# anand-12/botorch

Measured on AMD Instinct MI355X. Metric: acq-evals/sec (q x restarts x MC), qEI forward, higher is better.
Workload: dtype f64; 1 GPU; C3 qEI forward: SingleTaskGP n=4096 d=6, q=16, 512 restarts/GPU, 512 Sobol MC samples, best_f = max(Y) - 1.5; n=4096, d=6, q=16, restarts_per_gpu=512, mc=512, parallelism=restart-sharded x1

## Files before the change

botorch_amd/csrc/post.hip:

```cpp
#include "common.h"
#include "post_wide_sched.h"

#include <algorithm>
#include <atomic>
#include <cstdlib>
#include <map>
#include <mutex>
#include <tuple>
#include <vector>

namespace {

constexpr int PC = 128;
constexpr int PI = 128;
constexpr int PK = 16;
constexpr int PLD = 144;
constexpr int DP = 8;
constexpr int kSlots = 512;
constexpr int kTileDoubles = 32 * 64;
#ifndef KXT_K
#define KXT_K 16
#endif

template <int KIND, int ND>
__device__ __forceinline__ double eval_kernel_row(const double (&xi)[ND], const double* __restrict__ Xt,
                                                  int n, int k, double outputscale, bool ivalid) {
  if (k >= n || !ivalid) return 0.0;
  const double* xt = Xt + (int64_t)k * DP;
  double d2 = 0.0;
#pragma unroll
  for (int t = 0; t < ND; ++t) {
    const double df = xi[t] - xt[t];
    d2 = fma(df, df, d2);
  }
#ifdef BO_PROBE_CHEAP_KERNEL
  return outputscale * d2 * 0.0;
#else
  return outputscale * kernel_from_d2<KIND>(d2);
#endif
}

__host__ __device__ __forceinline__ int splitk_chunks(int ci, int n, int kc_len) {
  const int e = ci * PC + PC;
  const int kfull = n < e ? n : e;
  return (kfull + kc_len - 1) / kc_len;
}
__host__ __device__ __forceinline__ int64_t splitk_base(int ci, int n, int kc_len) {
  int64_t s = 0;
  for (int c = 0; c < ci; ++c) s += splitk_chunks(c, n, kc_len);
  return s;
}

__device__ __forceinline__ void post_store_rt(const v4d (&acc)[8], int ci, int row0, int lane,
                                              int nI, double* __restrict__ Rt) {
  const int c0 = ci * PC;
  const int nrows_pad = nI * PI;
#pragma unroll
  for (int ct = 0; ct < 8; ++ct)
#pragma unroll
    for (int r = 0; r < 4; ++r) {
      const int c = c0 + ct * 16 + mfma_row(lane, r);
      Rt[(int64_t)c * nrows_pad + row0 + mfma_col(lane)] = acc[ct][r];
    }
}

__device__ __forceinline__ void post_epilogue(const v4d (&acc)[8], int ci, int row0, int lane,
                                              int n, const double* __restrict__ beta, int nI,
                                              double* __restrict__ Spart,
                                              double* __restrict__ mpart) {
  const int c0 = ci * PC;
  const int nrows16 = nI * (PI / 16);
  const int nrows_pad = nI * PI;
  v4d P = v4d_zero();
#pragma unroll
  for (int ct = 0; ct < 8; ++ct)
#pragma unroll
    for (int r = 0; r < 4; ++r) P = mfma_f64(acc[ct][r], acc[ct][r], P);
  double* sp = Spart + ((int64_t)ci * nrows16 + row0 / 16) * 256;
#pragma unroll
  for (int r = 0; r < 4; ++r) sp[mfma_row(lane, r) * 16 + mfma_col(lane)] = P[r];

  double m = 0.0;
#pragma unroll
  for (int ct = 0; ct < 8; ++ct)
#pragma unroll
    for (int r = 0; r < 4; ++r) {
      const int c = c0 + ct * 16 + mfma_row(lane, r);
      m = fma(acc[ct][r], (c < n) ? beta[c] : 0.0, m);
    }
  m += __shfl_xor(m, 16);
  m += __shfl_xor(m, 32);
  if (lane < 16) mpart[(int64_t)ci * nrows_pad + row0 + lane] = m;
}

struct FusedDx {
  const double* dmean;
  const double* dcov;
  const double* alpha;
  const double* Xq;
  const double* Xt;
  double ystd, outputscale;
  int B, q, Qp;
  double* part;
};

constexpr int POST_MAXM = 8;
struct PostMembers {
  const double* U[POST_MAXM];
  const double* beta[POST_MAXM];
  const double* Kt[POST_MAXM];
  double* Spart[POST_MAXM];
  double* mpart[POST_MAXM];
  double* Rt[POST_MAXM];
  int nm;
};

#ifndef BO_POST_PAIRED_REV
#define BO_POST_PAIRED_REV 1
#endif
#ifndef BO_USTORE_ALWAYS
#define BO_USTORE_ALWAYS 1
#endif
#ifndef BO_POST_RING
#define BO_POST_RING 1
#endif
template <int KIND, int ND, bool SPLIT, bool CROSS, bool PRE = false, bool LOWERK = false,
          bool FUSEDX = false>
__global__ __launch_bounds__(256, 2) void post_partials_kernel(
    const double* __restrict__ Xq, int nrows, const double* __restrict__ Xt, int n,
    const double* __restrict__ U, int64_t ldu, const double* __restrict__ beta,
    double outputscale, int nC, int nI, double* __restrict__ Spart, double* __restrict__ mpart,
    double* __restrict__ Rt, const int4* __restrict__ segs, const int* __restrict__ wg_off,
    double* __restrict__ work, const double* __restrict__ Qc, int rq, int64_t ldq,
    double* __restrict__ Cx, const double* __restrict__ Kt, int grouped, FusedDx fx = FusedDx{},
    int rt_blk = 0, PostMembers pm = PostMembers{}) {
  constexpr bool RING = PRE && BO_POST_RING;
  __shared__ __attribute__((aligned(16))) double Us[RING ? 3 : 2][PK][PLD];
  __shared__ __attribute__((aligned(16))) double Ks[2][PK][PLD];

  const int bid = blockIdx.x;
  int ci = 0, ii = 0, kbeg = 0, kend = 0;
  int ci_long = 0, ci_short = 0;
  if constexpr (SPLIT) {
  } else if (grouped == 2) {
    const int xcd = bid & 7;
    const int slot = bid >> 3;
    const int t = (slot >> 6) * 8 + xcd;
    const int w = slot & 63;
    const int nIG = nI >> 3;
    const int p = t / nIG;
    if (p >= (nC >> 4)) return;
    ci_long = ((nC >> 3) - 1 - p) * 8 + 7 - (w & 7);
    ci_short = p * 8 + (w & 7);
    ii = (t % nIG) * 8 + (w >> 3);
  } else if (grouped) {
    const int xcd = bid & 7;
    const int slot = bid >> 3;
    const int t = (slot >> 6) * 8 + xcd;
    const int w = slot & 63;
    const int nIG = nI >> 3;
    const int cg = (nC >> 3) - 1 - t / nIG;
    if (cg < 0) return;
    ci = cg * 8 + 7 - (w & 7);
    ii = (t % nIG) * 8 + (w >> 3);
    kend = min(n, ci * PC + PC);
  } else {
    const int xcd = bid & 7;
    const int slot = bid >> 3;
    const int jj = slot / nI;
    ii = slot - jj * nI;
    const int pos = jj * 8 + xcd;
    if (pos >= nC) return;
    ci = nC - 1 - pos;
    kend = min(n, ci * PC + PC);
  }
  if (LOWERK && !SPLIT && grouped != 2) {
    ci = nC - 1 - ci;
    kbeg = ci * PC;
    kend = n;
  }
  const double* const U_all = U;
  const double* const beta_all = beta;
  const double* const Kt_all = Kt;
  double* const Spart_all = Spart;
  double* const mpart_all = mpart;
  double* const Rt_all = Rt;
  int sbeg = 0, send = 1;
  if constexpr (SPLIT) {
    sbeg = wg_off[bid];
    send = wg_off[bid + 1];
  } else {
    if (grouped == 2) send = 2;
// ... 454 lines not shown
  }}
#define BO_W_STORE(G)                                                              \
  {_Pragma("unroll") for (int e = 0; e < SS; ++e) {                               \
    double* dst = &Us[(G) & (postw::kStages - 1)][e * PK + wave][2 * lane];        \
    *reinterpret_cast<double2*>(dst) = make_double2(us_[e][0], us_[e][1]);         \
    *reinterpret_cast<double2*>(dst + 8 * PLD) = make_double2(us_[e][2], us_[e][3]); \
  }}
#define BO_W_LOAD_B(UNIT, DST)                                                     \
  {                                                                                \
    const int u_ = min(max((UNIT), 0), 2 * nsteps - 1);                            \
    const double* bp = bbase + (int64_t)postw::unit_step(u_) * bstep +             \
                       (int64_t)(postw::unit_slice0(u_) * 4) * ldk;                \
    _Pragma("unroll") for (int it = 0; it < 2; ++it)                              \
      _Pragma("unroll") for (int sl = 0; sl < 2; ++sl)                               \
        DST[it][sl] = bp[(int64_t)(4 * sl) * ldk + it * 16];                         \
  }
#define BO_W_UADDR(UNIT)                                                           \
  (&Us[postw::stage_of_step(postw::unit_step(UNIT))]                               \
      [postw::stage_row_of_step(postw::unit_step(UNIT), PK) +                      \
       postw::unit_slice0(UNIT) * 4 + (lane >> 4)][lane & 15])
#define BO_W_PREF(UNIT)                                                            \
  {                                                                                \
    const double* us = BO_W_UADDR(UNIT);                                           \
    _Pragma("unroll") for (int ct = 0; ct < 8; ++ct) an[ct] = us[ct * 16];        \
  }
#define BO_W_UNIT(UNIT, BOP, PREF, DIAG)                                           \
  {                                                                                \
    const double* us = BO_W_UADDR(UNIT);                                           \
    const int kd = kfirst + postw::unit_step(UNIT) * kdir - c0;                    \
    const int ctb = (DIAG) ? __builtin_amdgcn_readfirstlane(max(kd, 0) >> 4) : 0;  \
    _Pragma("unroll") for (int sl = 0; sl < 2; ++sl) {                             \
      double a[8];                                                                 \
      _Pragma("unroll") for (int ct = 0; ct < 8; ++ct)                            \
        a[ct] = ((PREF) && sl == 0) ? an[ct] : us[sl * 4 * PLD + ct * 16];         \
      _Pragma("unroll") for (int ct = 0; ct < 8; ++ct)                            \
        if (!(DIAG) || ct >= ctb) {                                                \
          _Pragma("unroll") for (int it = 0; it < 2; ++it)                        \
            acc[ct][it] = mfma_f64(a[ct], BOP[it][sl], acc[ct][it]);              \
        }                                                                          \
    }                                                                              \
  }
#define BO_W_INTERVAL(J, DIAG, GUARD, STORE)                                       \
  {                                                                                \
    const int u0 = NU * (J) - lag;                                                 \
    if (!late) BO_W_PREF(u0);   \
    _Pragma("unroll") for (int k = 0; k < NU; ++k) {                              \
      if (!(GUARD) || postw::unit_valid(u0 + k, nsteps))                           \
        BO_W_UNIT(u0 + k, bu[k & 1], k == 0, DIAG)                                 \
      BO_W_LOAD_B(u0 + k + 2, bu[k & 1]);                                          \
      if ((STORE) && k == postw::store_after_unit(true) && late) BO_W_STORE((J) + 1);  \
    }                                                                              \
    if (late) BO_W_PREF(u0 + NU);               \
    if ((STORE) && !late) BO_W_STORE((J) + 1);                                     \
    if (STORE) BO_W_LOAD_U((J) + 2);             \
    __syncthreads();                                                               \
  }
    static_assert(postw::unit_at(3, 1, false) == 3 * NU + 1 &&
                      postw::unit_at(3, 1, true) == 3 * NU + 1 - postw::kLag &&
                      postw::store_after_unit(false) == NU - 1,
                  "BO_W_INTERVAL's units and stores are post_wide_sched.h's");

    BO_W_LOAD_U(0);
#pragma unroll
    for (int k = 0; k < 2; ++k) BO_W_LOAD_B(k - lag, bu[k]);
    BO_W_STORE(0);
    BO_W_LOAD_U(1);
    __syncthreads();
    const int jfull = nsteps / SS;
    constexpr int LB = postw::kLag > 1 ? (postw::kLag + 1) / 2 : 1;
    const int jd0 = min(jfull, max(1, d0 / SS));
    const int jd1 = max(jd0, min(jfull, (d1 + LB - 1) / SS + 1));
    int j = 0;
    BO_W_INTERVAL(j, 1, 1, 1)
    for (j = 1; j < jd0; ++j) BO_W_INTERVAL(j, 0, 0, 1)
    for (; j < jd1; ++j) BO_W_INTERVAL(j, 1, 0, 1)
    for (; j < jfull; ++j) BO_W_INTERVAL(j, 0, 0, 1)
    if (j < nss) {
      BO_W_INTERVAL(j, 1, 1, 1)
    }
    BO_W_INTERVAL(nss, 1, 1, 0)
#undef BO_W_INTERVAL
#undef BO_W_UNIT
#undef BO_W_PREF
#undef BO_W_UADDR
#undef BO_W_LOAD_B
#undef BO_W_STORE
#undef BO_W_LOAD_U

    const int nrows_pad = nI * PI;
    if (Rt != nullptr && rt_blk) {
#pragma unroll
      for (int ct = 0; ct < 8; ++ct)
#pragma unroll
        for (int it = 0; it < 2; ++it) {
          double* blk = Rt + ((int64_t)((c0 >> 4) + ct) * nrows16 +
                              ((i0 + wave * 32 + it * 16) >> 4)) * 256 + lane;
#pragma unroll
          for (int r = 0; r < 4; ++r) blk[r * 64] = acc[ct][it][r];
        }
    } else if (Rt != nullptr) {
#pragma unroll
      for (int ct = 0; ct < 8; ++ct)
#pragma unroll
        for (int it = 0; it < 2; ++it)
#pragma unroll
          for (int r = 0; r < 4; ++r) {
            const int c = c0 + ct * 16 + mfma_row(lane, r);
            const int i = i0 + wave * 32 + it * 16 + mfma_col(lane);
            Rt[(int64_t)c * nrows_pad + i] = acc[ct][it][r];
          }
    }
#pragma unroll
    for (int it = 0; it < 2; ++it) {
      v4d P = v4d_zero();
#pragma unroll
      for (int ct = 0; ct < 8; ++ct)
#pragma unroll
        for (int r = 0; r < 4; ++r) P = mfma_f64(acc[ct][it][r], acc[ct][it][r], P);
      const int row0 = i0 + wave * 32 + it * 16;
      double* sp = Spart + ((int64_t)ci * nrows16 + row0 / 16) * 256;
#pragma unroll
      for (int r = 0; r < 4; ++r) sp[mfma_row(lane, r) * 16 + mfma_col(lane)] = P[r];
      double m = 0.0;
#pragma unroll
      for (int ct = 0; ct < 8; ++ct)
#pragma unroll
        for (int r = 0; r < 4; ++r) {
          const int c = c0 + ct * 16 + mfma_row(lane, r);
          m = fma(acc[ct][it][r], (c < n) ? beta[c] : 0.0, m);
        }
      m += __shfl_xor(m, 16);
      m += __shfl_xor(m, 32);
      if (lane < 16) mpart[(int64_t)ci * nrows_pad + row0 + lane] = m;
    }
  }
}

struct RowsFromX {
  const double* X;
  const double* ls;
  int B, q, d, Qp;
  double* Xq_out;
};

struct KxtMembers {
  const double* ls[8];
  const double* Xt[8];
  double os[8];
  double* Xq[8];
  double* Kt[8];
  int nm;
};

template <int KIND, int ND, int KK = KXT_K, bool FROMX = false>
__global__ __launch_bounds__(256) void kxt_build_kernel(const double* __restrict__ Xq, int nrows,
                                                        const double* __restrict__ Xt, int n,
                                                        int np, int nrows_pad, double outputscale,
                                                        double* __restrict__ Kt,
                                                        RowsFromX rx = RowsFromX{},
                                                        KxtMembers km = KxtMembers{}) {
  if (km.nm > 0) {
    const int m = blockIdx.z;
    rx.ls = km.ls[m];
    rx.Xq_out = km.Xq[m];
    Xt = km.Xt[m];
    outputscale = km.os[m];
    Kt = km.Kt[m];
  }
  const int i = blockIdx.x * 256 + threadIdx.x;
  const int k0 = blockIdx.y * KK;
  const bool iv = i < nrows;
  double xi[ND];
  if constexpr (FROMX) {
    const int b = i / rx.Qp, a = i - (i / rx.Qp) * rx.Qp;
    const bool real = iv && b < rx.B && a < rx.q;
#pragma unroll
    for (int t = 0; t < ND; ++t)
      xi[t] = (real && t < rx.d) ? rx.X[((int64_t)b * rx.q + a) * rx.d + t] / rx.ls[t] : 0.0;
    if (blockIdx.y == 0 && i < nrows_pad) {
#pragma unroll
      for (int t = 0; t < DP; ++t)
        rx.Xq_out[(int64_t)i * DP + t] =
            (real && t < rx.d) ? rx.X[((int64_t)b * rx.q + a) * rx.d + t] / rx.ls[t] : 0.0;
    }
  } else {
#pragma unroll
    for (int t = 0; t < ND; ++t) xi[t] = iv ? Xq[(int64_t)i * DP + t] : 0.0;
  }
  if (i >= nrows_pad) return;
#pragma unroll 4
  for (int kk = 0; kk < KK; ++kk) {
    const int k = k0 + kk;
    if (k < np) Kt[(int64_t)k * nrows_pad + i] = eval_kernel_row<KIND, ND>(xi, Xt, n, k, outputscale, iv);
  }
}

__global__ __launch_bounds__(256) void post_splitk_reduce_kernel(
    const double* __restrict__ work, const int4* __restrict__ red, int n, int nI,
    const double* __restrict__ beta_all, double* __restrict__ Spart_all,
    double* __restrict__ mpart_all, double* __restrict__ Rt_all, PostMembers pm = PostMembers{}) {
  __shared__ double part[3][32][64];
  const int4 r4 = red[blockIdx.x / (PI / 16)];
  const int sub = blockIdx.x % (PI / 16);
  const int ci = r4.x & 0xffffff, rt = r4.y * (PI / 16) + sub;
  const int mem = r4.x >> 24;
  const bool memb = pm.nm > 0;
  const double* beta = memb ? pm.beta[mem] : beta_all;
  double* Spart = memb ? pm.Spart[mem] : Spart_all;
  double* mpart = memb ? pm.mpart[mem] : mpart_all;
  double* Rt = memb ? pm.Rt[mem] : Rt_all;
  const int lane = threadIdx.x & 63;
  const int wave = threadIdx.x >> 6;
  v4d acc[8];
#pragma unroll
  for (int ct = 0; ct < 8; ++ct) acc[ct] = v4d_zero();
  const int cend = r4.z + r4.w;
  int c = r4.z + wave;
  for (; c + 4 < cend; c += 8) {
    const double* w0 = work + ((int64_t)c * (PI / 16) + sub) * kTileDoubles + lane;
    const double* w1 = w0 + 4 * (PI / 16) * kTileDoubles;
    double v0[32], v1[32];
#pragma unroll
    for (int e = 0; e < 32; ++e) {
      v0[e] = w0[e * 64];
      v1[e] = w1[e * 64];
    }
#pragma unroll
    for (int ct = 0; ct < 8; ++ct)
#pragma unroll
      for (int r = 0; r < 4; ++r) acc[ct][r] += v0[ct * 4 + r];
#pragma unroll
    for (int ct = 0; ct < 8; ++ct)
#pragma unroll
      for (int r = 0; r < 4; ++r) acc[ct][r] += v1[ct * 4 + r];
  }
  if (c < cend) {
    const double* w = work + ((int64_t)c * (PI / 16) + sub) * kTileDoubles + lane;
#pragma unroll
    for (int ct = 0; ct < 8; ++ct)
#pragma unroll
      for (int r = 0; r < 4; ++r) acc[ct][r] += w[(ct * 4 + r) * 64];
  }
  if (wave > 0) {
#pragma unroll
    for (int ct = 0; ct < 8; ++ct)
#pragma unroll
      for (int r = 0; r < 4; ++r) part[wave - 1][ct * 4 + r][lane] = acc[ct][r];
  }
  __syncthreads();
  if (wave != 0) return;
#pragma unroll
  for (int w = 0; w < 3; ++w)
#pragma unroll
    for (int ct = 0; ct < 8; ++ct)
#pragma unroll
      for (int r = 0; r < 4; ++r) acc[ct][r] += part[w][ct * 4 + r][lane];
  if (Rt != nullptr) post_store_rt(acc, ci, rt * 16, lane, nI, Rt);
  if (Spart != nullptr) post_epilogue(acc, ci, rt * 16, lane, n, beta, nI, Spart, mpart);
}

template <int KIND>
__global__ __launch_bounds__(256) void post_dx_reduce_kernel(
    const double* __restrict__ part, int nC, int nrows_pad, int q, int Qp, int d,
    const double* __restrict__ Xq, const double* __restrict__ dcov,
    const double* __restrict__ ls, double outputscale, double ystd, double* __restrict__ dX) {
  const int b = blockIdx.x;
  const int tid = threadIdx.x;
  if (tid >= q * d) return;
  const int a = tid / d, t = tid - (tid / d) * d;
  const int64_t row = (int64_t)b * Qp + a;
  double s = 0.0;
  for (int ci = 0; ci < nC; ++ci) s += part[((int64_t)ci * nrows_pad + row) * DP + t];
  const double s2 = ystd * ystd;
  for (int c = 0; c < q; ++c) {
    if (c == a) continue;
    const int64_t rc = (int64_t)b * Qp + c;
    double d2 = 0.0;
#pragma unroll
    for (int u = 0; u < DP; ++u) {
      const double df = Xq[row * DP + u] - Xq[rc * DP + u];
      d2 = fma(df, df, d2);
    }
    const double g = s2 * (dcov[((int64_t)b * q + a) * q + c] + dcov[((int64_t)b * q + c) * q + a]);
    s = fma(g * dkernel_factor<KIND>(d2, outputscale), Xq[row * DP + t] - Xq[rc * DP + t], s);
  }
  dX[((int64_t)b * q + a) * d + t] = s / ls[t];
}

__global__ void prepare_rows_kernel(const double* __restrict__ X, int B, int q, int d,
                                    int Qp, const double* __restrict__ ls, int nrows_pad,
                                    double* __restrict__ Xq) {
  const int64_t idx = (int64_t)blockIdx.x * blockDim.x + threadIdx.x;
  if (idx >= (int64_t)nrows_pad * DP) return;
  const int64_t row = idx / DP;
  const int t = (int)(idx % DP);
  const int64_t b = row / Qp;
  const int a = (int)(row % Qp);
  double v = 0.0;
  if (b < B && a < q && t < d) v = X[(b * q + a) * d + t] / ls[t];
  Xq[idx] = v;
}

constexpr int SMU = 32;
#ifndef SMALL_DEPTH
#define SMALL_DEPTH 2
#endif
#ifndef SMALL_PAIRED
#define SMALL_PAIRED 1
#endif
#ifndef SMALL_WAVES
#define SMALL_WAVES 8
#endif
constexpr int SMW = SMALL_WAVES;

__device__ __forceinline__ void small_load(const double* __restrict__ U, int64_t ldu,
                                           const double* __restrict__ Kt, int64_t ldk, int kb,
                                           int c0, int r0, int lane, double (&a)[4][2],
                                           double (&b)[4][2]) {
  const int kr = lane >> 4, cl = lane & 15;
#pragma unroll
  for (int ks = 0; ks < 4; ++ks) {
    const int64_t k = kb + 4 * ks + kr;
#pragma unroll
    for (int h = 0; h < 2; ++h) {
      a[ks][h] = U[k * ldu + c0 + 16 * h + cl];
      b[ks][h] = Kt[k * ldk + r0 + 16 * h + cl];
    }
  }
}

__device__ __forceinline__ void small_tile(const double* __restrict__ U, int64_t ldu,
                                           const double* __restrict__ Kt, int64_t ldk, int c0,
                                           int r0, int nsteps, int first, int lane,
                                           v4d (&acc)[2][2]) {
  double a0[4][2], b0[4][2], a1[4][2], b1[4][2];
  int s = first;
  if (s < nsteps) small_load(U, ldu, Kt, ldk, PK * s, c0, r0, lane, a0, b0);
  if (s + SMW < nsteps) small_load(U, ldu, Kt, ldk, PK * (s + SMW), c0, r0, lane, a1, b1);
#if SMALL_DEPTH >= 3
  double a2[4][2], b2[4][2];
  if (s + 2 * SMW < nsteps) small_load(U, ldu, Kt, ldk, PK * (s + 2 * SMW), c0, r0, lane, a2, b2);
  for (; s < nsteps; s += SMW) {
    double a3[4][2], b3[4][2];
    const bool more = s + 3 * SMW < nsteps;
    if (more) small_load(U, ldu, Kt, ldk, PK * (s + 3 * SMW), c0, r0, lane, a3, b3);
#pragma unroll
// ... 469 lines not shown
    const double np_ = (double)nC * PC;
    if ((double)B * Qp * np_ * np_ > 1.2e9) return BO_OK;
  }
  *nparts = (int)(ceil_div(n, PC) * PC / (2 * SMU));
  return BO_OK;
}

int bo_post_small_batched(int nm, const double* const* Kt, const double* const* U,
                          const double* const* beta, double* const* Spart, double* const* mpart,
                          double* const* Rt, int64_t B, int q, int64_t n, int64_t ldu,
                          void* stream) {
  int Qp, nrows_pad, nC;
  int s = bo_post_geometry(B, q, n, &Qp, &nrows_pad, &nC);
  if (s) return s;
  BO_CHECK_ARG(nm >= 1 && nm <= SMALL_MAXM, "bo_post_small_batched: %d models (1..%d)", nm,
               SMALL_MAXM);
  BO_CHECK_ARG(Kt && U && beta && Spart && mpart, "bo_post_small_batched: null pointer array");
  const int64_t np = (int64_t)nC * PC;
  BO_CHECK_ARG(ldu >= np, "bo_post_small: ldu %lld < padded order %lld", (long long)ldu,
               (long long)np);
  SmallArgs a{};
  for (int m = 0; m < nm; ++m) {
    BO_CHECK_ARG(Kt[m] && U[m] && beta[m] && Spart[m] && mpart[m], "bo_post_small: null buffer");
    a.m[m] = SmallMember{Kt[m], U[m], beta[m], Spart[m], mpart[m], Rt ? Rt[m] : nullptr};
  }
  if (B == 0) return BO_OK;
  a.ldk = nrows_pad;
  a.ldu = ldu;
  a.n = (int)n;
  a.nct = (int)(np / SMU);
  a.units = (int)(ceil_div(B * Qp, SMU) * (a.nct / 2));
  post_small_kernel<<<(unsigned)(a.units * nm), 64 * SMW, 0, as_stream(stream)>>>(a);
  BO_LAUNCH_CHECK();
  return BO_OK;
}

int bo_post_small(const double* Kt, int64_t B, int q, int64_t n, const double* U, int64_t ldu,
                  const double* beta, double* Spart, double* mpart, double* Rt, void* stream) {
  return bo_post_small_batched(1, &Kt, &U, &beta, &Spart, &mpart, &Rt, B, q, n, ldu, stream);
}

int bo_post_members_work(int nm, int64_t B, int q, int64_t n, int64_t* work_elems) {
  BO_CHECK_ARG(nm >= 1 && nm <= POST_MAXM, "bo_post_members_work: %d models (1..%d)", nm, POST_MAXM);
  int Qp, nrows_pad, nC;
  int s = bo_post_geometry(B, q, n, &Qp, &nrows_pad, &nC);
  if (s) return s;
  int kc = 0;
  int64_t we = 0;
  s = bo_post_split_plan(B, q, n, 0, &kc, &we);
  if (s) return s;
  *work_elems = -1;
  if (kc != -1 || nrows_pad == 0) return BO_OK;
  *work_elems = (int64_t)plan_chunks(nC, nrows_pad / PI, (int)n, -1, kSlots, PLAN_POST, nm) * PI * PC;
  return BO_OK;
}

int bo_post_partials_members(int nm, const double* const* Kt, const double* const* U,
                             const double* const* beta, double* const* Spart, double* const* mpart,
                             double* const* Rt, const double* Xq0, int64_t B, int q, int64_t n,
                             int64_t ldu, double* work, void* stream) {
  BO_CHECK_ARG(nm >= 1 && nm <= POST_MAXM, "bo_post_partials_members: %d models (1..%d)", nm,
               POST_MAXM);
  BO_CHECK_ARG(Kt && U && beta && Spart && mpart && Xq0, "bo_post_partials_members: null pointer");
  int Qp, nrows_pad, nC;
  int s = bo_post_geometry(B, q, n, &Qp, &nrows_pad, &nC);
  if (s) return s;
  if (nrows_pad == 0) return BO_OK;
  BO_CHECK_ARG(ldu % 2 == 0 && ldu >= (int64_t)nC * PC, "U leading dim %lld too small", (long long)ldu);
  int64_t we = 0;
  s = bo_post_members_work(nm, B, q, n, &we);
  if (s) return s;
  BO_CHECK_ARG(we >= 0, "bo_post_partials_members: the one-model plan is not stream-K here");
  BO_CHECK_ARG(we == 0 || work != nullptr, "bo_post_partials_members: workspace of %lld doubles needed",
               (long long)we);
  PostMembers pm{};
  pm.nm = nm;
  for (int m = 0; m < nm; ++m) {
    BO_CHECK_ARG(Kt[m] && U[m] && beta[m] && Spart[m] && mpart[m], "bo_post_partials_members: null buffer");
    pm.U[m] = U[m];
    pm.beta[m] = beta[m];
    pm.Kt[m] = Kt[m];
    pm.Spart[m] = Spart[m];
    pm.mpart[m] = mpart[m];
    pm.Rt[m] = Rt ? Rt[m] : nullptr;
  }
  const int nI = nrows_pad / PI;
  DevPlan* plan = nullptr;
  s = device_plan(nC, nI, (int)n, -1, &plan, PLAN_POST, nm);
  if (s) return s;
  hipStream_t st = as_stream(stream);
  post_partials_kernel<BO_RBF, 1, true, false, true><<<(unsigned)plan->W, 256, 0, st>>>(
      Xq0, B * Qp, nullptr, (int)n, U[0], ldu, beta[0], 1.0, nC, nI, Spart[0], mpart[0], nullptr,
      plan->segs, plan->wg_off, work, nullptr, 0, 0, nullptr, Kt[0], 0, FusedDx{}, 0, pm);
  BO_LAUNCH_CHECK();
  if (plan->nred > 0) {
    post_splitk_reduce_kernel<<<(unsigned)(plan->nred * (PI / 16)), 256, 0, st>>>(
        work, plan->red, (int)n, nI, beta[0], Spart[0], mpart[0], nullptr, pm);
    BO_LAUNCH_CHECK();
  }
  return BO_OK;
}

int bo_post_split_work(int64_t B, int q, int64_t n, int kc_len, int64_t* work_elems) {
  int Qp, nrows_pad, nC;
  int s = bo_post_geometry(B, q, n, &Qp, &nrows_pad, &nC);
  if (s) return s;
  *work_elems = 0;
  if (kc_len == 0 || nrows_pad == 0) return BO_OK;
  *work_elems = (int64_t)plan_chunks(nC, nrows_pad / PI, (int)n, kc_len, kSlots, PLAN_POST) * PI * PC;
  return BO_OK;
}

int bo_post_split_table(int64_t B, int q, int64_t n, int kc_len, int* segs, int cap, int* wg_off,
                        int wcap, int* nseg, int* nwg) {
  int Qp, nrows_pad, nC;
  int s = bo_post_geometry(B, q, n, &Qp, &nrows_pad, &nC);
  if (s) return s;
  BO_CHECK_ARG(kc_len != 0 && nrows_pad > 0, "bo_post_split_table: a split plan of a non-empty batch");
  const SplitPlan p = build_split_plan(nC, nrows_pad / PI, (int)n, kc_len, kSlots);
  *nseg = (int)p.segs.size();
  *nwg = (int)p.wg_off.size() - 1;
  for (int i = 0; i < *nseg && i < cap; ++i) {
    segs[4 * i] = p.segs[i].x;
    segs[4 * i + 1] = p.segs[i].y;
    segs[4 * i + 2] = p.segs[i].z;
    segs[4 * i + 3] = p.segs[i].w;
  }
  for (int i = 0; i <= *nwg && i <= wcap; ++i) wg_off[i] = p.wg_off[i];
  return BO_OK;
}

int bo_prepare_rows(const double* X, int B, int q, int d, const double* lengthscale,
                    double* Xq, void* stream) {
  BO_CHECK_ARG(d <= DP, "fused posterior kernel supports d <= %d (got %d)", DP, d);
  int Qp, nrows_pad, nC;
  int s = bo_post_geometry(B, q, 1, &Qp, &nrows_pad, &nC);
  if (s) return s;
  const int64_t tot = (int64_t)nrows_pad * DP;
  if (tot == 0) return BO_OK;
  prepare_rows_kernel<<<(unsigned)ceil_div(tot, 256), 256, 0, as_stream(stream)>>>(
      X, B, q, d, Qp, lengthscale, nrows_pad, Xq);
  BO_LAUNCH_CHECK();
  return BO_OK;
}

int bo_post_kxt(int kind, const double* Xq, int B, int q, int d, const double* Xt_scaled,
                int64_t n, double outputscale, double* Kt, void* stream) {
  BO_CHECK_ARG(kind == BO_RBF || kind == BO_MATERN52, "bad kernel kind %d", kind);
  BO_CHECK_ARG(d >= 1 && d <= DP, "fused posterior kernel supports 1 <= d <= %d", DP);
  int Qp, nrows_pad, nC;
  int s = bo_post_geometry(B, q, n, &Qp, &nrows_pad, &nC);
  if (s) return s;
  if (nrows_pad == 0) return BO_OK;
  const int np = nC * PC;
  const int nrows = B * Qp;
  hipStream_t st = as_stream(stream);
  const bool small = ceil_div(nrows_pad, 256) * ceil_div(np, KXT_K) < 1024;
  const dim3 grid((unsigned)ceil_div(nrows_pad, 256), (unsigned)ceil_div(np, small ? 2 : KXT_K));
#define BO_KXT(KIND, ND)                                                                        \
  if (small)                                                                                    \
    kxt_build_kernel<KIND, ND, 2><<<grid, 256, 0, st>>>(Xq, nrows, Xt_scaled, (int)n, np,       \
                                                        nrows_pad, outputscale, Kt);            \
  else                                                                                          \
    kxt_build_kernel<KIND, ND><<<grid, 256, 0, st>>>(Xq, nrows, Xt_scaled, (int)n, np, nrows_pad, \
                                                     outputscale, Kt)
#define BO_KXT_D(KIND)                       \
  switch (d) {                               \
    case 1: BO_KXT(KIND, 1); break;          \
    case 2: BO_KXT(KIND, 2); break;          \
    case 3: BO_KXT(KIND, 3); break;          \
    case 4: BO_KXT(KIND, 4); break;          \
    case 5: BO_KXT(KIND, 5); break;          \
    case 6: BO_KXT(KIND, 6); break;          \
    default: BO_KXT(KIND, 8); break;         \
  }
  if (kind == BO_RBF) {
    BO_KXT_D(BO_RBF)
  } else {
    BO_KXT_D(BO_MATERN52)
  }
#undef BO_KXT_D
#undef BO_KXT
  BO_LAUNCH_CHECK();
  return BO_OK;
}

static int kxt_small_k() {
  static const int k = [] {
    const char* e = std::getenv("BO_KXT_SMALL");
    const int v = e ? std::atoi(e) : 2;
    return (v == 1 || v == 2 || v == 4 || v == 8) ? v : 2;
  }();
  return k;
}

int bo_post_kxt_rows_members(int nm, int kind, const double* X, int B, int q, int d,
                             const double* const* lengthscale, const double* const* Xt_scaled,
                             const double* outputscale, int64_t n, double* const* Xq,
                             double* const* Kt, void* stream) {
  BO_CHECK_ARG(nm >= 1 && nm <= 8, "bo_post_kxt_rows_members: %d models (1..8)", nm);
  BO_CHECK_ARG(kind == BO_RBF || kind == BO_MATERN52, "bad kernel kind %d", kind);
  BO_CHECK_ARG(d >= 1 && d <= DP, "fused posterior kernel supports 1 <= d <= %d", DP);
  int Qp, nrows_pad, nC;
  int s = bo_post_geometry(B, q, n, &Qp, &nrows_pad, &nC);
  if (s) return s;
  if (nrows_pad == 0) return BO_OK;
  BO_CHECK_ARG(X && lengthscale && Xt_scaled && outputscale && Xq && Kt,
               "bo_post_kxt_rows_members: null pointer");
  KxtMembers km{};
  km.nm = nm;
  for (int m = 0; m < nm; ++m) {
    BO_CHECK_ARG(lengthscale[m] && Xt_scaled[m] && Xq[m] && Kt[m], "bo_post_kxt_rows_members: null buffer");
    km.ls[m] = lengthscale[m];
    km.Xt[m] = Xt_scaled[m];
    km.os[m] = outputscale[m];
    km.Xq[m] = Xq[m];
    km.Kt[m] = Kt[m];
  }
  const int np = nC * PC;
  const int nrows = B * Qp;
  hipStream_t st = as_stream(stream);
  const RowsFromX rx{X, lengthscale[0], B, q, d, Qp, Xq[0]};
  const bool small = ceil_div(nrows_pad, 256) * ceil_div(np, KXT_K) * nm < 1024;
  const int kk = small ? kxt_small_k() : KXT_K;
  const dim3 grid((unsigned)ceil_div(nrows_pad, 256), (unsigned)ceil_div(np, kk), (unsigned)nm);
#define BO_KXTM_K(KIND, ND, K)                                                                 \
  kxt_build_kernel<KIND, ND, K, true><<<grid, 256, 0, st>>>(nullptr, nrows, Xt_scaled[0], (int)n, \
                                                            np, nrows_pad, outputscale[0], Kt[0], rx, km)
#define BO_KXTM(KIND, ND)                  \
  switch (kk) {                            \
    case 1: BO_KXTM_K(KIND, ND, 1); break; \
    case 2: BO_KXTM_K(KIND, ND, 2); break; \
    case 4: BO_KXTM_K(KIND, ND, 4); break; \
    case 8: BO_KXTM_K(KIND, ND, 8); break; \
    default: BO_KXTM_K(KIND, ND, KXT_K); break; \
  }
#define BO_KXTM_D(KIND)                      \
  switch (d) {                               \
    case 1: BO_KXTM(KIND, 1); break;         \
    case 2: BO_KXTM(KIND, 2); break;         \
    case 3: BO_KXTM(KIND, 3); break;         \
    case 4: BO_KXTM(KIND, 4); break;         \
    case 5: BO_KXTM(KIND, 5); break;         \
    case 6: BO_KXTM(KIND, 6); break;         \
    default: BO_KXTM(KIND, 8); break;        \
  }
  if (kind == BO_RBF) {
    BO_KXTM_D(BO_RBF)
  } else {
    BO_KXTM_D(BO_MATERN52)
  }
#undef BO_KXTM_D
#undef BO_KXTM
#undef BO_KXTM_K
  BO_LAUNCH_CHECK();
  return BO_OK;
}

int bo_post_kxt_rows(int kind, const double* X, int B, int q, int d, const double* lengthscale,
                     const double* Xt_scaled, int64_t n, double outputscale, double* Xq, double* Kt,
                     void* stream) {
  BO_CHECK_ARG(kind == BO_RBF || kind == BO_MATERN52, "bad kernel kind %d", kind);
  BO_CHECK_ARG(d >= 1 && d <= DP, "fused posterior kernel supports 1 <= d <= %d", DP);
  int Qp, nrows_pad, nC;
  int s = bo_post_geometry(B, q, n, &Qp, &nrows_pad, &nC);
  if (s) return s;
  if (nrows_pad == 0) return BO_OK;
  BO_CHECK_ARG(X && lengthscale && Xt_scaled && Xq && Kt, "bo_post_kxt_rows: null buffer");
  const int np = nC * PC;
  const int nrows = B * Qp;
  hipStream_t st = as_stream(stream);
  const RowsFromX rx{X, lengthscale, B, q, d, Qp, Xq};
  const bool small = ceil_div(nrows_pad, 256) * ceil_div(np, KXT_K) < 1024;
  const int kk = small ? kxt_small_k() : KXT_K;
  const dim3 grid((unsigned)ceil_div(nrows_pad, 256), (unsigned)ceil_div(np, kk));
#define BO_KXTR_K(KIND, ND, K)                                                                 \
  kxt_build_kernel<KIND, ND, K, true><<<grid, 256, 0, st>>>(nullptr, nrows, Xt_scaled, (int)n,  \
                                                            np, nrows_pad, outputscale, Kt, rx)
#define BO_KXTR(KIND, ND)                  \
  switch (kk) {                            \
    case 1: BO_KXTR_K(KIND, ND, 1); break; \
    case 2: BO_KXTR_K(KIND, ND, 2); break; \
    case 4: BO_KXTR_K(KIND, ND, 4); break; \
    case 8: BO_KXTR_K(KIND, ND, 8); break; \
    default: BO_KXTR_K(KIND, ND, KXT_K); break; \
  }
#define BO_KXTR_D(KIND)                      \
  switch (d) {                               \
    case 1: BO_KXTR(KIND, 1); break;         \
    case 2: BO_KXTR(KIND, 2); break;         \
    case 3: BO_KXTR(KIND, 3); break;         \
    case 4: BO_KXTR(KIND, 4); break;         \
    case 5: BO_KXTR(KIND, 5); break;         \
    case 6: BO_KXTR(KIND, 6); break;         \
    default: BO_KXTR(KIND, 8); break;        \
  }
  if (kind == BO_RBF) {
    BO_KXTR_D(BO_RBF)
  } else {
    BO_KXTR_D(BO_MATERN52)
  }
#undef BO_KXTR_D
#undef BO_KXTR
#undef BO_KXTR_K
  BO_LAUNCH_CHECK();
  return BO_OK;
}

int bo_post_partials_impl(const BoPostPartialsArgs* a, void* stream) {
  const int kc_len = a->kc_len;
  const int64_t n = a->n;
  const bool blocked = a->rt_layout == BO_RT_BLOCKED;
  BO_CHECK_ARG(a->rt_layout == BO_RT_ROWMAJOR || (blocked && kc_len == 0 && !a->Qc),
               "rt_layout %d: the blocked R^T is stored by one-pass grids without a cross term",
               a->rt_layout);
  BO_CHECK_ARG(a->Qc == nullptr || (kc_len == 0 && a->rq >= 1 && a->rq <= 16 && a->ldq >= n &&
                                    a->Cx != nullptr),
               "cross term: one-pass only, 1 <= rq <= 16 rows (got %d), ldq >= n, Cx given", a->rq);
  BO_CHECK_ARG(a->kind == BO_RBF || a->kind == BO_MATERN52, "bad kernel kind %d", a->kind);
  BO_CHECK_ARG(a->ldu % 2 == 0 && a->ldu >= ceil_div(n, PC) * PC, "U leading dim %lld too small",
               (long long)a->ldu);
  if (a->B == 0) return BO_OK;
  const bool pre = a->Kt != nullptr;
  BO_CHECK_ARG(kc_len == 0 || kc_len == -1 || (kc_len > 0 && kc_len % PK == 0),
               "split chunk %d must be 0, -1 (stream-K) or a positive multiple of %d", kc_len, PK);
  int Qp, nrows_pad, nC;
  int s = bo_post_geometry(a->B, a->q, n, &Qp, &nrows_pad, &nC);
  if (s) return s;
  const int nI = nrows_pad / PI;
  const int nrows = a->B * Qp;
  if (nI == 0) return BO_OK;
  BO_CHECK_ARG(a->d >= 1 && a->d <= DP, "fused posterior kernel supports 1 <= d <= %d", DP);
  const int grouped = (kc_len == 0 && nC % 8 == 0 && nI % 8 == 0)
                          ? ((nC % 16 == 0 && paired_enabled()) ? 2 : 1) : 0;
  DevPlan* plan = nullptr;
  if (kc_len != 0) {
    s = device_plan(nC, nI, (int)n, kc_len, &plan);
    if (s) return s;
    BO_CHECK_ARG(plan->nchunks == 0 || a->work != nullptr, "split plan needs a workspace of %lld doubles",
                 (long long)plan->nchunks * PI * PC);
  }
  const int64_t blocks = kc_len != 0    ? plan->W
                         : grouped == 2 ? 512 * (int64_t)ceil_div((nC / 16) * (nI / 8), 8)
                         : grouped      ? 512 * (int64_t)ceil_div((nC / 8) * (nI / 8), 8)
                                        : 8 * ceil_div(nC, 8) * (int64_t)nI;
  const int4* segs = plan ? plan->segs : nullptr;
  const int* wg_off = plan ? plan->wg_off : nullptr;
  hipStream_t st = as_stream(stream);
  if (wide_applies(nC, nI, kc_len, a->Qc != nullptr, pre)) {
    const int64_t wblocks = 256 * (int64_t)ceil_div((nC / 16) * (nI / 8), 8);
    post_partials_wide_kernel<<<(unsigned)wblocks, 512, 0, st>>>(
        (int)n, a->U, a->ldu, a->beta, nC, nI, a->Spart, a->mpart, a->Rt, a->Kt, blocked);
    BO_LAUNCH_CHECK();
    return BO_OK;
  }
#define BO_POST_GO(KIND, ND, SPL, CRS, PRE_)                                                \
  post_partials_kernel<KIND, ND, SPL, CRS, PRE_><<<(unsigned)blocks, 256, 0, st>>>(          \
      a->Xq, nrows, a->Xt_scaled, (int)n, a->U, a->ldu, a->beta, a->outputscale, nC, nI,    \
      a->Spart, a->mpart, a->Rt, segs, wg_off, a->work, a->Qc, a->rq, a->ldq, a->Cx, a->Kt, \
      grouped, FusedDx{}, blocked)
#define BO_POST_LAUNCH(KIND, ND)                                                            \
  if (kc_len != 0) {                                                                        \
    if (pre) BO_POST_GO(KIND, ND, true, false, true);                                       \
    else BO_POST_GO(KIND, ND, true, false, false);                                          \
  } else if (a->Qc != nullptr) {                                                            \
    if (pre) BO_POST_GO(KIND, ND, false, true, true);                                     \
    else BO_POST_GO(KIND, ND, false, true, false);                                          \
  } else {                                                                                  \
    if (pre) BO_POST_GO(KIND, ND, false, false, true);                                      \
    else BO_POST_GO(KIND, ND, false, false, false);                                         \
  }
#define BO_POST_DISPATCH_D(KIND)                   \
  switch (a->d) {                                  \
    case 1: BO_POST_LAUNCH(KIND, 1); break;        \
    case 2: BO_POST_LAUNCH(KIND, 2); break;        \
    case 3: BO_POST_LAUNCH(KIND, 3); break;        \
    case 4: BO_POST_LAUNCH(KIND, 4); break;        \
    case 5: BO_POST_LAUNCH(KIND, 5); break;        \
    case 6: BO_POST_LAUNCH(KIND, 6); break;        \
    default: BO_POST_LAUNCH(KIND, 8); break;       \
  }
  if (a->kind == BO_RBF) {
    BO_POST_DISPATCH_D(BO_RBF)
  } else {
    BO_POST_DISPATCH_D(BO_MATERN52)
  }
#undef BO_POST_DISPATCH_D
#undef BO_POST_LAUNCH
#undef BO_POST_GO
  BO_LAUNCH_CHECK();
  if (plan && plan->nred > 0) {
    post_splitk_reduce_kernel<<<(unsigned)(plan->nred * (PI / 16)), 256, 0, st>>>(
        a->work, plan->red, (int)n, nI, a->beta, a->Spart, a->mpart, a->Rt);
    BO_LAUNCH_CHECK();
  }
  return BO_OK;
}

int bo_post_set_wide(int mode) {
  BO_CHECK_ARG(mode >= -1 && mode <= 1, "bo_post_set_wide: mode %d (-1, 0 or 1)", mode);
  wide_mode().store(mode);
  return BO_OK;
}

int bo_post_wide_applies(int64_t B, int q, int64_t n, int kc_len, int has_cross, int has_kt,
                         int* out) {
  int Qp, nrows_pad, nC;
  int s = bo_post_geometry(B, q, n, &Qp, &nrows_pad, &nC);
  if (s) return s;
  *out = wide_applies(nC, nrows_pad / PI, kc_len, has_cross != 0, has_kt != 0) ? 1 : 0;
  return BO_OK;
}

int bo_post_wide_schedule(int nsteps, int half, int rev, int cap, int* n_barriers, int* n_events,
                          int* events) {
  BO_CHECK_ARG(nsteps >= 1 && (half == 0 || half == 1) && n_barriers && n_events,
               "bo_post_wide_schedule: nsteps %d, half %d", nsteps, half);
  const bool late = half == 1;
  const int lag = postw::lag_of(late);
  int ne = 0;
  auto emit = [&](int j, int kind, int step, int slice) {
    if (events && ne < cap) {
      int* e = events + 6 * (int64_t)ne;
      e[0] = j; e[1] = kind; e[2] = step; e[3] = slice; e[4] = postw::stage_of_step(step);
      e[5] = postw::walk_k0(step, nsteps, rev != 0, PK);
    }
    ++ne;
  };
  auto first_read = [&](int j, int u) {
    if (postw::unit_valid(u, nsteps)) emit(j, 0, postw::unit_step(u), postw::unit_slice0(u));
  };
  auto store = [&](int j) {
    const int g = postw::store_superstep(j, nsteps);
    for (int e = 0; g >= 0 && e < postw::kSS; ++e) emit(j, 1, g * postw::kSS + e, -1);
  };
  for (int e = 0; e < postw::kSS; ++e) emit(-1, 1, e, -1);
  for (int j = 0; j < postw::intervals(nsteps); ++j) {
    if (!postw::prefetches(lag > 0)) first_read(j, postw::unit_at(j, 0, late));
    for (int k = 0; k < postw::kNU; ++k) {
      const int u = postw::unit_at(j, k, late);
      if (postw::unit_valid(u, nsteps)) {
        for (int i = 0; i < postw::kSlices / 2; ++i) {
          const int sl = postw::unit_slice0(u) + i;
          if (!(k == 0 && i == 0)) emit(j, 0, postw::unit_step(u), sl);
          emit(j, 2, postw::unit_step(u), sl);
        }
      }
      if (lag > 0 && k == postw::store_after_unit(true)) store(j);
    }
    if (postw::prefetches(lag > 0) && j + 1 < postw::intervals(nsteps))
      first_read(j, postw::unit_at(j + 1, 0, late));
    if (lag == 0) store(j);
  }
  *n_barriers = postw::barriers(nsteps);
  *n_events = ne;
  return BO_OK;
}
// ... 221 lines not shown
```

Baseline: 2.021 billion acq-evals/s.

## Stage training points in LDS and compute two rows per thread in Kxt build

Rewrites the K(x, X_train) build kernel so each block stages its chunk of training points in shared memory, and each thread computes two adjacent query rows and writes them with 16-byte vector stores. The k-chunk grows from 16 to 32. The k<np bounds check is dropped and the FROMX row decode uses shift/mask, which assumes Qp is a power of two. The intent is to cut redundant global loads of Xt and store instructions in a kernel bound by memory writes. In exchange the change adds a shared-memory sync and new alignment and size preconditions, and consolidates the launch code into shared helpers.

```diff
diff --git a/botorch_amd/csrc/post.hip b/botorch_amd/csrc/post.hip
--- a/botorch_amd/csrc/post.hip
+++ b/botorch_amd/csrc/post.hip
@@ -19,8 +19,28 @@
 constexpr int kSlots = 512;
 constexpr int kTileDoubles = 32 * 64;
 #ifndef KXT_K
-#define KXT_K 16
+#define KXT_K 32
 #endif
+#ifndef KXT_ROWS
+#define KXT_ROWS 2
+#endif
+#ifndef KXT_UNROLL
+#define KXT_UNROLL 2
+#endif
+#ifndef KXT_STAGE_LDS
+#define KXT_STAGE_LDS 1
+#endif
+constexpr int kKxtSmallUnit = 16;
+typedef double v2d __attribute__((ext_vector_type(2)));
+
+template <int KIND>
+__device__ __forceinline__ double scaled_kernel_value(double d2, double outputscale) {
+#ifdef BO_PROBE_CHEAP_KERNEL
+  return outputscale * d2 * 0.0;
+#else
+  return outputscale * kernel_from_d2<KIND>(d2);
+#endif
+}
 
 template <int KIND, int ND>
 __device__ __forceinline__ double eval_kernel_row(const double (&xi)[ND], const double* __restrict__ Xt,
@@ -33,11 +53,7 @@
     const double df = xi[t] - xt[t];
     d2 = fma(df, df, d2);
   }
-#ifdef BO_PROBE_CHEAP_KERNEL
-  return outputscale * d2 * 0.0;
-#else
-  return outputscale * kernel_from_d2<KIND>(d2);
-#endif
+  return scaled_kernel_value<KIND>(d2, outputscale);
 }
 
 __host__ __device__ __forceinline__ int splitk_chunks(int ci, int n, int kc_len) {
@@ -798,13 +814,17 @@
   int nm;
 };
 
-template <int KIND, int ND, int KK = KXT_K, bool FROMX = false>
+template <int KIND, int ND, int KK, bool FROMX, int ROWS>
 __global__ __launch_bounds__(256) void kxt_build_kernel(const double* __restrict__ Xq, int nrows,
                                                         const double* __restrict__ Xt, int n,
-                                                        int np, int nrows_pad, double outputscale,
+                                                        int nrows_pad, double outputscale,
                                                         double* __restrict__ Kt,
                                                         RowsFromX rx = RowsFromX{},
                                                         KxtMembers km = KxtMembers{}) {
+  static_assert(PC % KK == 0, "np = nC * PC is a whole number of k-chunks: no k < np test");
+  static_assert(ROWS == 1 || ROWS == 2, "one row, or two adjacent rows and 16-byte stores");
+  constexpr int NST = (KK * DP + 255) / 256;
+  __shared__ double xts[KK * DP];
   if (km.nm > 0) {
     const int m = blockIdx.z;
     rx.ls = km.ls[m];
@@ -813,31 +833,156 @@
     outputscale = km.os[m];
     Kt = km.Kt[m];
   }
-  const int i = blockIdx.x * 256 + threadIdx.x;
   const int k0 = blockIdx.y * KK;
-  const bool iv = i < nrows;
-  double xi[ND];
+  double stage[NST];
+#pragma unroll
+  for (int s = 0; s < NST; ++s) {
+    const int e = s * 256 + threadIdx.x;
+    const int k = min(k0 + e / DP, n - 1);
+    stage[s] = (NST * 256 == KK * DP || e < KK * DP) ? Xt[(int64_t)k * DP + e % DP] : 0.0;
+  }
+  const int i0 = (blockIdx.x * 256 + threadIdx.x) * ROWS;
+  bool iv[ROWS];
+  double xi[ROWS][ND];
   if constexpr (FROMX) {
-    const int b = i / rx.Qp, a = i - (i / rx.Qp) * rx.Qp;
-    const bool real = iv && b < rx.B && a < rx.q;
-#pragma unroll
-    for (int t = 0; t < ND; ++t)
-      xi[t] = (real && t < rx.d) ? rx.X[((int64_t)b * rx.q + a) * rx.d + t] / rx.ls[t] : 0.0;
-    if (blockIdx.y == 0 && i < nrows_pad) {
-#pragma unroll
-      for (int t = 0; t < DP; ++t)
-        rx.Xq_out[(int64_t)i * DP + t] =
-            (real && t < rx.d) ? rx.X[((int64_t)b * rx.q + a) * rx.d + t] / rx.ls[t] : 0.0;
+    const int sh = __ffs(rx.Qp) - 1;
+    double xr[ROWS][ND], lsv[ND];
+    bool real[ROWS];
+#pragma unroll
+    for (int r = 0; r < ROWS; ++r) {
+      const int i = i0 + r;
+      iv[r] = i < nrows;
+      const int b = i >> sh, a = i & (rx.Qp - 1);
+      real[r] = iv[r] && b < rx.B && a < rx.q;
+      const double* xrow = rx.X + (real[r] ? ((int64_t)b * rx.q + a) * rx.d : 0);
+#pragma unroll
+      for (int t = 0; t < ND; ++t) xr[r][t] = xrow[t < rx.d ? t : 0];
+    }
+#pragma unroll
+    for (int t = 0; t < ND; ++t) lsv[t] = rx.ls[t < rx.d ? t : 0];
+    asm volatile("" ::: "memory");
+#pragma unroll
+    for (int r = 0; r < ROWS; ++r)
+#pragma unroll
+      for (int t = 0; t < ND; ++t) xi[r][t] = (real[r] && t < rx.d) ? xr[r][t] / lsv[t] : 0.0;
+    if (blockIdx.y == 0) {
+#pragma unroll
+      for (int r = 0; r < ROWS; ++r)
+        if (i0 + r < nrows_pad) {
+#pragma unroll
+          for (int t = 0; t < DP; ++t)
+            rx.Xq_out[(int64_t)(i0 + r) * DP + t] = t < ND ? xi[r][t < ND ? t : 0] : 0.0;
+        }
     }
   } else {
 #pragma unroll
-    for (int t = 0; t < ND; ++t) xi[t] = iv ? Xq[(int64_t)i * DP + t] : 0.0;
-  }
-  if (i >= nrows_pad) return;
-#pragma unroll 4
+    for (int r = 0; r < ROWS; ++r) {
+      iv[r] = i0 + r < nrows;
+#pragma unroll
+      for (int t = 0; t < ND; ++t) xi[r][t] = iv[r] ? Xq[(int64_t)(i0 + r) * DP + t] : 0.0;
+    }
+  }
+#pragma unroll
+  for (int s = 0; s < NST; ++s) {
+    const int e = s * 256 + threadIdx.x;
+    if (NST * 256 == KK * DP || e < KK * DP) xts[e] = stage[s];
+  }
+  __syncthreads();
+  if (i0 >= nrows_pad) return;
+  double* out = Kt + (int64_t)k0 * nrows_pad + i0;
+#pragma unroll KXT_UNROLL
   for (int kk = 0; kk < KK; ++kk) {
-    const int k = k0 + kk;
-    if (k < np) Kt[(int64_t)k * nrows_pad + i] = eval_kernel_row<KIND, ND>(xi, Xt, n, k, outputscale, iv);
+    const bool kv = k0 + kk < n;
+    double v[ROWS];
+#pragma unroll
+    for (int r = 0; r < ROWS; ++r) {
+      double d2 = 0.0;
+#pragma unroll
+      for (int t = 0; t < ND; ++t) {
+#if KXT_STAGE_LDS
+        const double df = xi[r][t] - xts[kk * DP + t];
+#else
+        const double df = xi[r][t] - Xt[(int64_t)min(k0 + kk, n - 1) * DP + t];
+#endif
+        d2 = fma(df, df, d2);
+      }
+      const double val = scaled_kernel_value<KIND>(d2, outputscale);
+      v[r] = (kv && iv[r]) ? val : 0.0;
+    }
+    if constexpr (ROWS == 2) {
+      v2d w;
+      w.x = v[0];
+      w.y = v[1];
+      *reinterpret_cast<v2d*>(out) = w;
+    } else {
+      *out = v[0];
+    }
+    out += nrows_pad;
+  }
+}
+
+static int kxt_small_k() {
+  static const int k = [] {
+    const char* e = std::getenv("BO_KXT_SMALL");
+    const int v = e ? std::atoi(e) : 2;
+    return (v == 1 || v == 2 || v == 4 || v == 8) ? v : 2;
+  }();
+  return k;
+}
+
+struct KxtLaunch {
+  int nrows_pad, np, nrows, n;
+  hipStream_t st;
+};
+struct KxtShape {
+  int kk, rows;
+};
+static bool kxt_aligned16(const void* p) { return (reinterpret_cast<uintptr_t>(p) & 15) == 0; }
+static KxtShape kxt_shape(const KxtLaunch& L, int nm, int small_k, bool aligned16) {
+  const bool small = ceil_div(L.nrows_pad, 256) * ceil_div(L.np, kKxtSmallUnit) * nm < 1024;
+  if (small) return KxtShape{small_k, 1};
+  const bool two = aligned16 && KXT_ROWS == 2 &&
+                   ceil_div(L.nrows_pad, 512) * (L.np / KXT_K) * nm >= 2048;
+  return KxtShape{KXT_K, two ? 2 : 1};
+}
+
+template <int KIND, int ND, bool FROMX>
+static void kxt_launch(KxtShape sh, const KxtLaunch& L, const double* Xq, const double* Xt,
+                       double outputscale, double* Kt, const RowsFromX& rx, const KxtMembers& km) {
+  const dim3 grid((unsigned)ceil_div(L.nrows_pad, 256 * sh.rows), (unsigned)(L.np / sh.kk),
+                  (unsigned)(km.nm > 0 ? km.nm : 1));
+#define BO_KXT_LAUNCH(K, R)                                                              \
+  kxt_build_kernel<KIND, ND, K, FROMX, R><<<grid, 256, 0, L.st>>>(Xq, L.nrows, Xt, L.n, \
+                                                                  L.nrows_pad, outputscale, Kt, rx, km)
+  if (sh.rows == 2) {
+    BO_KXT_LAUNCH(KXT_K, 2);
+  } else if (sh.kk == 2) {
+    BO_KXT_LAUNCH(2, 1);
+  } else if (sh.kk == KXT_K) {
+    BO_KXT_LAUNCH(KXT_K, 1);
+  } else if constexpr (FROMX) {
+    if (sh.kk == 1) {
+      BO_KXT_LAUNCH(1, 1);
+    } else if (sh.kk == 4) {
+      BO_KXT_LAUNCH(4, 1);
+    } else {
+      BO_KXT_LAUNCH(8, 1);
+    }
+  }
+#undef BO_KXT_LAUNCH
+}
+
+template <int KIND, bool FROMX>
+static void kxt_launch_d(int d, KxtShape sh, const KxtLaunch& L, const double* Xq, const double* Xt,
+                         double outputscale, double* Kt, const RowsFromX& rx, const KxtMembers& km) {
+  switch (d) {
+    case 1: kxt_launch<KIND, 1, FROMX>(sh, L, Xq, Xt, outputscale, Kt, rx, km); break;
+    case 2: kxt_launch<KIND, 2, FROMX>(sh, L, Xq, Xt, outputscale, Kt, rx, km); break;
+    case 3: kxt_launch<KIND, 3, FROMX>(sh, L, Xq, Xt, outputscale, Kt, rx, km); break;
+    case 4: kxt_launch<KIND, 4, FROMX>(sh, L, Xq, Xt, outputscale, Kt, rx, km); break;
+    case 5: kxt_launch<KIND, 5, FROMX>(sh, L, Xq, Xt, outputscale, Kt, rx, km); break;
+    case 6: kxt_launch<KIND, 6, FROMX>(sh, L, Xq, Xt, outputscale, Kt, rx, km); break;
+    default: kxt_launch<KIND, 8, FROMX>(sh, L, Xq, Xt, outputscale, Kt, rx, km); break;
   }
 }
 
@@ -1613,46 +1758,14 @@
   int s = bo_post_geometry(B, q, n, &Qp, &nrows_pad, &nC);
   if (s) return s;
   if (nrows_pad == 0) return BO_OK;
-  const int np = nC * PC;
-  const int nrows = B * Qp;
-  hipStream_t st = as_stream(stream);
-  const bool small = ceil_div(nrows_pad, 256) * ceil_div(np, KXT_K) < 1024;
-  const dim3 grid((unsigned)ceil_div(nrows_pad, 256), (unsigned)ceil_div(np, small ? 2 : KXT_K));
-#define BO_KXT(KIND, ND)                                                                        \
-  if (small)                                                                                    \
-    kxt_build_kernel<KIND, ND, 2><<<grid, 256, 0, st>>>(Xq, nrows, Xt_scaled, (int)n, np,       \
-                                                        nrows_pad, outputscale, Kt);            \
-  else                                                                                          \
-    kxt_build_kernel<KIND, ND><<<grid, 256, 0, st>>>(Xq, nrows, Xt_scaled, (int)n, np, nrows_pad, \
-                                                     outputscale, Kt)
-#define BO_KXT_D(KIND)                       \
-  switch (d) {                               \
-    case 1: BO_KXT(KIND, 1); break;          \
-    case 2: BO_KXT(KIND, 2); break;          \
-    case 3: BO_KXT(KIND, 3); break;          \
-    case 4: BO_KXT(KIND, 4); break;          \
-    case 5: BO_KXT(KIND, 5); break;          \
-    case 6: BO_KXT(KIND, 6); break;          \
-    default: BO_KXT(KIND, 8); break;         \
-  }
-  if (kind == BO_RBF) {
-    BO_KXT_D(BO_RBF)
-  } else {
-    BO_KXT_D(BO_MATERN52)
-  }
-#undef BO_KXT_D
-#undef BO_KXT
+  const KxtLaunch L{nrows_pad, nC * PC, B * Qp, (int)n, as_stream(stream)};
+  const KxtShape sh = kxt_shape(L, 1, 2, kxt_aligned16(Kt));
+  if (kind == BO_RBF)
+    kxt_launch_d<BO_RBF, false>(d, sh, L, Xq, Xt_scaled, outputscale, Kt, RowsFromX{}, KxtMembers{});
+  else
+    kxt_launch_d<BO_MATERN52, false>(d, sh, L, Xq, Xt_scaled, outputscale, Kt, RowsFromX{}, KxtMembers{});
   BO_LAUNCH_CHECK();
   return BO_OK;
-}
-
-static int kxt_small_k() {
-  static const int k = [] {
-    const char* e = std::getenv("BO_KXT_SMALL");
-    const int v = e ? std::atoi(e) : 2;
-    return (v == 1 || v == 2 || v == 4 || v == 8) ? v : 2;
-  }();
-  return k;
 }
 
 int bo_post_kxt_rows_members(int nm, int kind, const double* X, int B, int q, int d,
@@ -1678,42 +1791,15 @@
     km.Xq[m] = Xq[m];
     km.Kt[m] = Kt[m];
   }
-  const int np = nC * PC;
-  const int nrows = B * Qp;
-  hipStream_t st = as_stream(stream);
+  const KxtLaunch L{nrows_pad, nC * PC, B * Qp, (int)n, as_stream(stream)};
   const RowsFromX rx{X, lengthscale[0], B, q, d, Qp, Xq[0]};
-  const bool small = ceil_div(nrows_pad, 256) * ceil_div(np, KXT_K) * nm < 1024;
-  const int kk = small ? kxt_small_k() : KXT_K;
-  const dim3 grid((unsigned)ceil_div(nrows_pad, 256), (unsigned)ceil_div(np, kk), (unsigned)nm);
-#define BO_KXTM_K(KIND, ND, K)                                                                 \
-  kxt_build_kernel<KIND, ND, K, true><<<grid, 256, 0, st>>>(nullptr, nrows, Xt_scaled[0], (int)n, \
-                                                            np, nrows_pad, outputscale[0], Kt[0], rx, km)
-#define BO_KXTM(KIND, ND)                  \
-  switch (kk) {                            \
-    case 1: BO_KXTM_K(KIND, ND, 1); break; \
-    case 2: BO_KXTM_K(KIND, ND, 2); break; \
-    case 4: BO_KXTM_K(KIND, ND, 4); break; \
-    case 8: BO_KXTM_K(KIND, ND, 8); break; \
-    default: BO_KXTM_K(KIND, ND, KXT_K); break; \
-  }
-#define BO_KXTM_D(KIND)                      \
-  switch (d) {                               \
-    case 1: BO_KXTM(KIND, 1); break;         \
-    case 2: BO_KXTM(KIND, 2); break;         \
-    case 3: BO_KXTM(KIND, 3); break;         \
-    case 4: BO_KXTM(KIND, 4); break;         \
-    case 5: BO_KXTM(KIND, 5); break;         \
-    case 6: BO_KXTM(KIND, 6); break;         \
-    default: BO_KXTM(KIND, 8); break;        \
-  }
-  if (kind == BO_RBF) {
-    BO_KXTM_D(BO_RBF)
-  } else {
-    BO_KXTM_D(BO_MATERN52)
-  }
-#undef BO_KXTM_D
-#undef BO_KXTM
-#undef BO_KXTM_K
+  bool aligned16 = true;
+  for (int m = 0; m < nm; ++m) aligned16 = aligned16 && kxt_aligned16(Kt[m]);
+  const KxtShape sh = kxt_shape(L, nm, kxt_small_k(), aligned16);
+  if (kind == BO_RBF)
+    kxt_launch_d<BO_RBF, true>(d, sh, L, nullptr, Xt_scaled[0], outputscale[0], Kt[0], rx, km);
+  else
+    kxt_launch_d<BO_MATERN52, true>(d, sh, L, nullptr, Xt_scaled[0], outputscale[0], Kt[0], rx, km);
   BO_LAUNCH_CHECK();
   return BO_OK;
 }
@@ -1728,42 +1814,13 @@
   if (s) return s;
   if (nrows_pad == 0) return BO_OK;
   BO_CHECK_ARG(X && lengthscale && Xt_scaled && Xq && Kt, "bo_post_kxt_rows: null buffer");
-  const int np = nC * PC;
-  const int nrows = B * Qp;
-  hipStream_t st = as_stream(stream);
+  const KxtLaunch L{nrows_pad, nC * PC, B * Qp, (int)n, as_stream(stream)};
   const RowsFromX rx{X, lengthscale, B, q, d, Qp, Xq};
-  const bool small = ceil_div(nrows_pad, 256) * ceil_div(np, KXT_K) < 1024;
-  const int kk = small ? kxt_small_k() : KXT_K;
-  const dim3 grid((unsigned)ceil_div(nrows_pad, 256), (unsigned)ceil_div(np, kk));
-#define BO_KXTR_K(KIND, ND, K)                                                                 \
-  kxt_build_kernel<KIND, ND, K, true><<<grid, 256, 0, st>>>(nullptr, nrows, Xt_scaled, (int)n,  \
-                                                            np, nrows_pad, outputscale, Kt, rx)
-#define BO_KXTR(KIND, ND)                  \
-  switch (kk) {                            \
-    case 1: BO_KXTR_K(KIND, ND, 1); break; \
-    case 2: BO_KXTR_K(KIND, ND, 2); break; \
-    case 4: BO_KXTR_K(KIND, ND, 4); break; \
-    case 8: BO_KXTR_K(KIND, ND, 8); break; \
-    default: BO_KXTR_K(KIND, ND, KXT_K); break; \
-  }
-#define BO_KXTR_D(KIND)                      \
-  switch (d) {                               \
-    case 1: BO_KXTR(KIND, 1); break;         \
-    case 2: BO_KXTR(KIND, 2); break;         \
-    case 3: BO_KXTR(KIND, 3); break;         \
-    case 4: BO_KXTR(KIND, 4); break;         \
-    case 5: BO_KXTR(KIND, 5); break;         \
-    case 6: BO_KXTR(KIND, 6); break;         \
-    default: BO_KXTR(KIND, 8); break;        \
-  }
-  if (kind == BO_RBF) {
-    BO_KXTR_D(BO_RBF)
-  } else {
-    BO_KXTR_D(BO_MATERN52)
-  }
-#undef BO_KXTR_D
-#undef BO_KXTR
-#undef BO_KXTR_K
+  const KxtShape sh = kxt_shape(L, 1, kxt_small_k(), kxt_aligned16(Kt));
+  if (kind == BO_RBF)
+    kxt_launch_d<BO_RBF, true>(d, sh, L, nullptr, Xt_scaled, outputscale, Kt, rx, KxtMembers{});
+  else
+    kxt_launch_d<BO_MATERN52, true>(d, sh, L, nullptr, Xt_scaled, outputscale, Kt, rx, KxtMembers{});
   BO_LAUNCH_CHECK();
   return BO_OK;
 }
```

New measurement: 2.044 billion acq-evals/s, median of 6. +1.1%, better.
